# raphaelsulzer/dgnn

Hardware: AMD Instinct MI355X
Metric: tetrahedra/sec (in/out classified), 1M-tet graph at 1/2/4/8 MI355X (higher is better)
Workload: dtype f32 (fp16x2-split products, 22-bit operands; `exact_f32` = bit-faithful fp32 products)

## Files before the change

### dgnn_amd/csrc/fused_ws.hip

```cpp
#include <stdlib.h>

#include "common.h"
#include "fused_common.h"

namespace {
using namespace fused;

typedef float f32x4_t __attribute__((ext_vector_type(4)));
#define H8(v) __builtin_bit_cast(f16x8, v)

constexpr int WS_C = 128;
constexpr int WS_TILE = 32;
constexpr int WS_NP = 8;
template <int CIN> struct WsC {
    static constexpr int NCH = CIN / 16;
    static constexpr int NV = NCH / 4;
    static constexpr int KH = CIN / 32;
    static constexpr int PP = CIN / 8;
    static constexpr int ROWB = 8 * CIN;
    static constexpr int SLOT = WS_TILE * ROWB;
    static constexpr int BP = NCH * 2 * 48 * 16;
};
template <int CIN, int RING> struct WsL {
    static constexpr int OFF_BP = RING * WsC<CIN>::SLOT;
    static constexpr int OFF_ROWF = OFF_BP + WsC<CIN>::BP;
    static constexpr int OFF_CST = OFF_ROWF + RING * WS_TILE * 4;
    static constexpr int OFF_SC = OFF_CST + 3 * WS_C * 4;
    static constexpr int OFF_DC = OFF_SC + 16 + 2 * RING * 4 + 16 + 16;
    static constexpr int OFF_PLOG = OFF_DC + (64 + 64 + 128 + 4) * 4;
    static constexpr int OFF_YS = OFF_PLOG + 2 * 4 * 32 * 8;
    static constexpr int OFF_CMAX = OFF_YS + 2 * 32 * 4;
    static constexpr int OFF_W0S = OFF_CMAX + 4 * 32 * 4;
    static constexpr int OFF_W0 = (OFF_W0S + 32 + 255) & ~255;
    static constexpr int OFF_YT = OFF_W0 + 4 * 4 * 2 * 64 * 16;
    static constexpr int SMEM = OFF_SC + 16 + 2 * RING * 4 + 16 + 16;
    static constexpr int SMEM_DEC = OFF_YT + 2 * 4 * 2 * 2 * 64 * 16;
    static_assert(SMEM_DEC <= 160 * 1024, "the LDS of one CU");
};

struct WsDec {
    const float* W0;
    const float* b0;
    const float* scale1;
    const float* shift1;
    const float* W3;
    const float* b3;
    float* logits;
};


__device__ __forceinline__ void st_nt16(float* p, f32x4_t v) { __builtin_nontemporal_store(v, reinterpret_cast<f32x4_t*>(p)); }
typedef uint32_t u32x2_t __attribute__((ext_vector_type(2)));
__device__ __forceinline__ float ub16_lo(uint32_t u) { return __builtin_fabsf(__builtin_bit_cast(float, u << 15)); }
__device__ __forceinline__ float ub16_hi(uint32_t u) { return __builtin_bit_cast(float, (u >> 16) << 15); }
__device__ __forceinline__ uint32_t ub16_enc(float v) {
    const uint32_t b = __builtin_bit_cast(uint32_t, v) & 0x7FFFFFFFu;
    return (b + 0x3FFFu + ((b >> 15) & 1u)) >> 15;
}
__device__ __forceinline__ uint32_t bits(float f) { return __builtin_bit_cast(uint32_t, f); }

constexpr int WS_KNOBS = 1 | (0 << 4);
template <int CIN, int RING, bool DEC, bool IO16 = false>
__global__ void __launch_bounds__(1024) k_sage_fused_ws(const int32_t* __restrict__ rowptr, const int32_t* __restrict__ src, const int32_t* __restrict__ eid,
                                                        int64_t n_dst, const float* __restrict__ x, const float* __restrict__ xdst, int64_t ldx,
                                                        const float* __restrict__ ea, int64_t lde, const float* __restrict__ We, const float* __restrict__ be,
                                                        const float* __restrict__ Wj, const float* __restrict__ bj, const float* __restrict__ Wi,
                                                        const float* __restrict__ scale, const float* __restrict__ shift, int relu, float* __restrict__ out,
                                                        int64_t ldo, int64_t ntiles, int knobs, WsDec dec) {
    static_assert(CIN == 128 || (CIN == 64 && !DEC), "input widths of the shipped model's 128-wide layers");
    static_assert(!IO16 || !DEC, "the decoder-carrying launch of the bf16-storage chain stays with fused_bf16.hip");
    const uint16_t* const x16 = reinterpret_cast<const uint16_t*>(x);
    const uint16_t* const xdst16 = reinterpret_cast<const uint16_t*>(xdst);
    uint16_t* const out16 = reinterpret_cast<uint16_t*>(out);
    typedef WsC<CIN> G;
    constexpr int NCH = G::NCH, NV = G::NV, KH = G::KH, PP = G::PP;
    extern __shared__ __attribute__((aligned(16))) char ws_smem[];
    const bool nt_store = (knobs & 1) != 0;
    typedef WsL<CIN, RING> L;
    char* const ring = ws_smem;
    char* const bpbuf = ws_smem + L::OFF_BP;
    float* const rowf = reinterpret_cast<float*>(ws_smem + L::OFF_ROWF);
    float* const cst = reinterpret_cast<float*>(ws_smem + L::OFF_CST);
    uint32_t* const scbuf = reinterpret_cast<uint32_t*>(ws_smem + L::OFF_SC);
    volatile uint32_t* const ready = reinterpret_cast<volatile uint32_t*>(ws_smem + L::OFF_SC + 16);
    volatile uint32_t* const done = ready + RING;
    volatile uint32_t* const ycnt = done + RING;
    volatile uint32_t* const yfree = ycnt + 2;
    volatile uint32_t* const lcnt = ycnt + 4;
    volatile uint32_t* const ccnt = ycnt + 6;
    float* const dcst = reinterpret_cast<float*>(ws_smem + L::OFF_DC);
    float* const plog = reinterpret_cast<float*>(ws_smem + L::OFF_PLOG);
    float* const ysc = reinterpret_cast<float*>(ws_smem + L::OFF_YS);
    uint32_t* const cmax = reinterpret_cast<uint32_t*>(ws_smem + L::OFF_CMAX);
    uint32_t* const w0max = reinterpret_cast<uint32_t*>(ws_smem + L::OFF_W0S);
    float* const w0inv = reinterpret_cast<float*>(ws_smem + L::OFF_W0S + 16);
    char* const w0buf = ws_smem + L::OFF_W0;
    char* const ytile = ws_smem + L::OFF_YT;
    typedef __attribute__((address_space(3))) volatile uint32_t lds_vu32;
    auto wait_for = [&](volatile uint32_t* ctr, uint32_t target) {
        asm volatile("" ::: "memory");
        lds_vu32* c3 = (lds_vu32*)ctr;
        while ((int32_t)(__builtin_amdgcn_readfirstlane((int)*c3) - (int)target) < 0) __builtin_amdgcn_s_sleep(1);
        asm volatile("" ::: "memory");
    };
    const int lane = lane_id(), w = wave_id_uniform();
    const int jcol = lane & 15, tq = lane >> 4;

    const int nwg = gridDim.x, xcd = blockIdx.x & 7, slot_ = blockIdx.x >> 3, wg_per_xcd = (nwg + 7 - xcd) >> 3;
    const int64_t per = (ntiles + 7) / 8, t_lo = xcd * per, t_hi = min(ntiles, t_lo + per);
    int64_t my_n = 0;
    if (t_lo + slot_ < t_hi) my_n = (t_hi - t_lo - slot_ + wg_per_xcd - 1) / wg_per_xcd;
    auto tile_of = [&](int64_t it) { return t_lo + slot_ + it * wg_per_xcd; };

    if (threadIdx.x == 0) scbuf[0] = 0u;
    if (threadIdx.x < 2 * RING + 8) ready[threadIdx.x] = 0u;
    if constexpr (DEC) {
        for (int n_ = threadIdx.x; n_ < 64; n_ += blockDim.x) {
            const float s1 = dec.scale1 ? dec.scale1[n_] : 1.f, h1 = dec.scale1 ? dec.shift1[n_] : 0.f;
            dcst[n_] = s1;
            dcst[64 + n_] = __fmaf_rn(dec.b0[n_], s1, h1);
            dcst[128 + n_] = dec.W3[n_];
            dcst[192 + n_] = dec.W3[64 + n_];
        }
        if (threadIdx.x < 2) dcst[256 + threadIdx.x] = dec.b3[threadIdx.x];
        if (threadIdx.x < 4 * WS_TILE) cmax[threadIdx.x] = 0u;
        if (threadIdx.x < 4) w0max[threadIdx.x] = 0u;
    }
    __syncthreads();
    if constexpr (DEC) {
#pragma unroll
        for (int hb = 0; hb < 4; ++hb) {
            uint32_t m0 = 0u;
            for (int e = threadIdx.x; e < 16 * WS_C; e += blockDim.x) m0 = umax(m0, absbits(dec.W0[hb * 16 * WS_C + e]));
            m0 = wave_umax(m0);
            if ((threadIdx.x & 63) == 0) atomicMax(&w0max[hb], m0);
        }
    }
    {
        uint32_t me = 0u;
        for (int e = threadIdx.x; e < CIN * FE; e += blockDim.x) me = umax(me, absbits(We[e]));
        for (int e = threadIdx.x; e < CIN; e += blockDim.x) me = umax(me, absbits(be[e]));
        me = wave_umax(me);
        if (lane == 0) atomicMax(&scbuf[0], me);
    }
    for (int c = threadIdx.x; c < WS_C; c += blockDim.x) {
        cst[c] = bj ? bj[c] : 0.f;
        cst[WS_C + c] = scale ? scale[c] : 1.f;
        cst[2 * WS_C + c] = scale ? shift[c] : 0.f;
    }
    __syncthreads();
    float sWe, inv_sWe;
    pow2_scales(scbuf[0], sWe, inv_sWe);
    constexpr bool LINE_OWN = !IO16 && NV == 2;
    auto chan = [](int j, int cb) { return LINE_OWN ? ((cb >> 2) * 64 + 4 * j + (cb & 3)) : NCH * j + cb; };
    for (int e = threadIdx.x; e < NCH * 48; e += blockDim.x) {
        const int cb = e / 48, gj = e - cb * 48, g = gj >> 4, j = gj & 15;
        const int c = chan(j, cb);
        uint32_t ph[4], pl[4];
#pragma unroll
        for (int d = 0; d < 4; ++d) {
            float v[2];
#pragma unroll
            for (int u = 0; u < 2; ++u) {
                const int k = 8 * g + 2 * d + u;
                v[u] = k < FE ? We[(int64_t)c * FE + k] : (k == FE ? be[c] : 0.f);
            }
            split2h(v[0] * sWe, v[1] * sWe, ph[d], pl[d]);
        }
        uint4* dst = reinterpret_cast<uint4*>(bpbuf + ((cb * 2) * 48 + gj) * 16);
        dst[0] = make_uint4(ph[0], ph[1], ph[2], ph[3]);
        dst[48] = make_uint4(pl[0], pl[1], pl[2], pl[3]);
    }

    auto stage_b = [&](uint32_t t, int hb, int b) {
        wait_for(ycnt + (t & 1), 8u * (t / 2 + 1));
        int ln = lane;
        asm volatile("" : "+v"(ln));
        const char* yt = ytile + ((t & 1) << 14) + ((b * 128 + ln) << 4);
        const char* wp = w0buf + ((hb * 512 + ln) << 4);
        const float inv = ysc[(t & 1) * WS_TILE + 16 * b + (ln & 15)] * w0inv[hb];
        f32x4_t hs = {0.f, 0.f, 0.f, 0.f};
#pragma unroll
        for (int s = 0; s < 4; ++s) {
            const f16x8 w0h = H8(*reinterpret_cast<const uint4*>(wp + (s << 11))), w0l = H8(*reinterpret_cast<const uint4*>(wp + (s << 11) + 1024));
            const f16x8 yh = H8(*reinterpret_cast<const uint4*>(yt + (s << 12))), yl = H8(*reinterpret_cast<const uint4*>(yt + (s << 12) + 1024));
            hs = __builtin_amdgcn_mfma_f32_16x16x32_f16(w0l, yh, hs, 0, 0, 0);
            hs = __builtin_amdgcn_mfma_f32_16x16x32_f16(w0h, yl, hs, 0, 0, 0);
            hs = __builtin_amdgcn_mfma_f32_16x16x32_f16(w0h, yh, hs, 0, 0, 0);
        }
        asm volatile("s_waitcnt lgkmcnt(0)" ::: "memory");
        if (lane == 0) atomicAdd(const_cast<uint32_t*>(yfree + (t & 1)), 1u);
#pragma unroll
        for (int i = 0; i < 4; ++i) hs[i] *= inv;
        const int u0 = 16 * hb + 4 * (ln >> 4);
        float l0 = 0.f, l1 = 0.f;
#pragma unroll
        for (int i = 0; i < 4; ++i) {
            const float hv = fmaxf(__fmaf_rn(hs[i], dcst[u0 + i], dcst[64 + u0 + i]), 0.f);
            l0 = __fmaf_rn(hv, dcst[128 + u0 + i], l0);
            l1 = __fmaf_rn(hv, dcst[192 + u0 + i], l1);
        }
        l0 = cross_row_sum(l0);
        l1 = cross_row_sum(l1);
        if (ln < 16) *reinterpret_cast<float2*>(plog + (((t & 1) * 4 + hb) * WS_TILE + 16 * b + ln) * 2) = make_float2(l0, l1);
        asm volatile("s_waitcnt lgkmcnt(0)" ::: "memory");
        if (lane == 0) atomicAdd(const_cast<uint32_t*>(lcnt + (t & 1)), 1u);
    };

    const int bsel = (knobs >> 4) & 3;
    auto b_on_consumers = [&](uint32_t t) { return bsel == 0 ? false : bsel == 1 ? (t & 1) == 0 : bsel == 2 ? (t & 3) != 3 : true; };

    if (w >= WS_NP) {
        const int cw = w - WS_NP;
        const int col = 16 * cw + jcol;
        uint32_t mw = 0u;
#pragma unroll
        for (int s = 0; s < 2 * KH; ++s) {
            const float* wr = (s < KH ? Wj : Wi) + (int64_t)col * CIN + 32 * (s % KH) + 8 * tq;
            const f32x4_t r0 = *reinterpret_cast<const f32x4_t*>(wr), r1 = *reinterpret_cast<const f32x4_t*>(wr + 4);
#pragma unroll
            for (int i = 0; i < 4; ++i) mw = umax(mw, umax(absbits(r0[i]), absbits(r1[i])));
        }
        float sW, inv_sW;
        pow2_scales(wave_umax(mw), sW, inv_sW);
        f16x8 wh[2 * KH], wl[2 * KH];
#pragma unroll
        for (int s = 0; s < 2 * KH; ++s) {
            const float* wr = (s < KH ? Wj : Wi) + (int64_t)col * CIN + 32 * (s % KH) + 8 * tq;
            const f32x4_t r0 = *reinterpret_cast<const f32x4_t*>(wr), r1 = *reinterpret_cast<const f32x4_t*>(wr + 4);
            uint32_t ph[4], pl[4];
            split2h(r0[0] * sW, r0[1] * sW, ph[0], pl[0]);
            split2h(r0[2] * sW, r0[3] * sW, ph[1], pl[1]);
            split2h(r1[0] * sW, r1[1] * sW, ph[2], pl[2]);
            split2h(r1[2] * sW, r1[3] * sW, ph[3], pl[3]);
            wh[s] = pack8h(ph);
            wl[s] = pack8h(pl);
        }
        if constexpr (DEC) {
#pragma unroll
            for (int u = 0; u < 2; ++u) {
                const int hb = 2 * (cw & 1) + u, ks = cw >> 1;
                float sW0, inv_sW0;
                pow2_scales(w0max[hb], sW0, inv_sW0);
                if (ks == 0 && lane == 0) w0inv[hb] = inv_sW0;
                const float* wr = dec.W0 + (int64_t)(16 * hb + jcol) * WS_C + 32 * ks + 8 * tq;
                const f32x4_t r0 = *reinterpret_cast<const f32x4_t*>(wr), r1 = *reinterpret_cast<const f32x4_t*>(wr + 4);
                uint32_t ph[4], pl[4];
                split2h(r0[0] * sW0, r0[1] * sW0, ph[0], pl[0]);
                split2h(r0[2] * sW0, r0[3] * sW0, ph[1], pl[1]);
                split2h(r1[0] * sW0, r1[1] * sW0, ph[2], pl[2]);
                split2h(r1[2] * sW0, r1[3] * sW0, ph[3], pl[3]);
                uint4* dst = reinterpret_cast<uint4*>(w0buf + (((hb * 4 + ks) * 128 + lane) << 4));
                dst[0] = make_uint4(ph[0], ph[1], ph[2], ph[3]);
                dst[64] = make_uint4(pl[0], pl[1], pl[2], pl[3]);
            }
        }
        __syncthreads();
        const int c0 = 16 * cw + 4 * tq;
        const int64_t n_it = my_n + (DEC ? 3 : 0);
        f32x4_t yp[2] = {{0.f, 0.f, 0.f, 0.f}, {0.f, 0.f, 0.f, 0.f}}, yn[2] = {yp[0], yp[1]};
        for (int64_t it = 1; it <= n_it; ++it) {
            if constexpr (DEC) {
                if (cw == 0 && it >= 4) {
                    const uint32_t t = (uint32_t)(it - 4);
                    wait_for(lcnt + (t & 1), 8u * (t / 2 + 1));
                    if (lane < WS_TILE) {
                        float s0 = dcst[256], s1 = dcst[257];
#pragma unroll
                        for (int q = 0; q < 4; ++q) {
                            const float* pq = plog + (((t & 1) * 4 + q) * WS_TILE + lane) * 2;
                            s0 += pq[0];
                            s1 += pq[1];
                        }
                        const int64_t cell = tile_of(t) * WS_TILE + lane;
                        if (cell < n_dst) *reinterpret_cast<float2*>(dec.logits + cell * 2) = make_float2(s0, s1);
                    }
                }
            }
            if (it >= 1 && it <= my_n) {
                const int sl = (int)((it - 1) % RING);
                wait_for(ready + sl, (uint32_t)(WS_NP * ((it - 1) / RING + 1)));
                const char* tb = ring + sl * G::SLOT;
                f32x4_t acc[2] = {{0.f, 0.f, 0.f, 0.f}, {0.f, 0.f, 0.f, 0.f}};
                int key = jcol;
                asm volatile("" : "+v"(key));
                f16x8 xh[2][2], xl[2][2];
                auto ld_step = [&](int s, int set) {
#pragma unroll
                    for (int b = 0; b < 2; ++b) {
                        const char* rp = tb + (16 * b + jcol) * G::ROWB;
                        xh[set][b] = H8(*reinterpret_cast<const uint4*>(rp + (((4 * s + tq) ^ key) << 4)));
                        xl[set][b] = H8(*reinterpret_cast<const uint4*>(rp + (((2 * PP + 4 * s + tq) ^ key) << 4)));
                    }
                };
                ld_step(0, 0);
#pragma unroll
                for (int s = 0; s < 2 * KH; ++s) {
                    const int set = s & 1;
                    if (s + 1 < 2 * KH) ld_step(s + 1, set ^ 1);
                    __builtin_amdgcn_sched_barrier(0);
#pragma unroll
                    for (int b = 0; b < 2; ++b) acc[b] = __builtin_amdgcn_mfma_f32_16x16x32_f16(wl[s], xh[set][b], acc[b], 0, 0, 0);
#pragma unroll
                    for (int b = 0; b < 2; ++b) acc[b] = __builtin_amdgcn_mfma_f32_16x16x32_f16(wh[s], xl[set][b], acc[b], 0, 0, 0);
#pragma unroll
                    for (int b = 0; b < 2; ++b) acc[b] = __builtin_amdgcn_mfma_f32_16x16x32_f16(wh[s], xh[set][b], acc[b], 0, 0, 0);
                    __builtin_amdgcn_sched_barrier(0);
                }
                float invr[2];
#pragma unroll
                for (int b = 0; b < 2; ++b) invr[b] = rowf[sl * WS_TILE + 16 * b + jcol] * inv_sW;
                asm volatile("s_waitcnt lgkmcnt(0)" ::: "memory");
                if (lane == 0) atomicAdd(const_cast<uint32_t*>(done + sl), 1u);
                const f32x4_t bb = *reinterpret_cast<const f32x4_t*>(cst + c0), sc = *reinterpret_cast<const f32x4_t*>(cst + WS_C + c0),
                              sh = *reinterpret_cast<const f32x4_t*>(cst + 2 * WS_C + c0);
                f32x4_t yv[2];
#pragma unroll
                for (int b = 0; b < 2; ++b) {
#pragma unroll
                    for (int i = 0; i < 4; ++i) {
                        float t_ = __fmaf_rn(acc[b][i], invr[b], bb[i]);
                        t_ = __fmaf_rn(t_, sc[i], sh[i]);
                        yv[b][i] = relu ? fmaxf(t_, 0.f) : t_;
                    }
                }
                if constexpr (!DEC) {
                    const int64_t cell0 = tile_of(it - 1) * WS_TILE;
#pragma unroll
                    for (int b = 0; b < 2; ++b) {
                        const int64_t cell = cell0 + 16 * b + jcol;
                        if (cell < n_dst) {
                            if constexpr (IO16) {
                                const u32x2_t pk = {ub16_enc(yv[b][0]) | (ub16_enc(yv[b][1]) << 16), ub16_enc(yv[b][2]) | (ub16_enc(yv[b][3]) << 16)};
                                if (nt_store) __builtin_nontemporal_store(pk, reinterpret_cast<u32x2_t*>(out16 + cell * ldo + c0));
                                else *reinterpret_cast<u32x2_t*>(out16 + cell * ldo + c0) = pk;
                            } else {
                                if (nt_store) st_nt16(out + cell * ldo + c0, yv[b]);
                                else *reinterpret_cast<f32x4_t*>(out + cell * ldo + c0) = yv[b];
                            }
                        }
                    }
                } else {
                    const uint32_t t = (uint32_t)(it - 1);
                    uint32_t* cm = cmax + (t & 3) * WS_TILE + jcol;
#pragma unroll
                    for (int b = 0; b < 2; ++b) {
                        const float my = fmaxf(fmaxf(fabsf(yv[b][0]), fabsf(yv[b][1])), fmaxf(fabsf(yv[b][2]), fabsf(yv[b][3])));
                        atomicMax(cm + 16 * b, ((t / 4 + 1) << 8) | (bits(my) >> 23));
                    }
                    asm volatile("s_waitcnt lgkmcnt(0)" ::: "memory");
                    if (lane == 0) atomicAdd(const_cast<uint32_t*>(ccnt + (t & 1)), 1u);
                    yn[0] = yv[0], yn[1] = yv[1];
                }
            }
            if constexpr (DEC) {
                if (it >= 2 && it <= my_n + 1) {
                    const uint32_t t = (uint32_t)(it - 2);
                    wait_for(ccnt + (t & 1), 8u * (t / 2 + 1));
                    wait_for(yfree + (t & 1), 8u * (t / 2));
                    int ln = lane;
                    asm volatile("" : "+v"(ln));
                    const uint32_t* cm = cmax + (t & 3) * WS_TILE + (ln & 15);
                    char* yt = ytile + ((t & 1) << 14) + ((cw >> 1) << 12) + (((ln & 15) + 16 * (2 * (cw & 1) + (ln >> 5))) << 4) + (((ln >> 4) & 1) << 3);
#pragma unroll
                    for (int b = 0; b < 2; ++b) {
                        float sY, inv_sY;
                        pow2_scales((cm[16 * b] & 255u) << 23, sY, inv_sY);
                        uint32_t ph[2], pl[2];
                        split2h(yp[b][0] * sY, yp[b][1] * sY, ph[0], pl[0]);
                        split2h(yp[b][2] * sY, yp[b][3] * sY, ph[1], pl[1]);
                        *reinterpret_cast<uint2*>(yt + (b << 11)) = make_uint2(ph[0], ph[1]);
                        *reinterpret_cast<uint2*>(yt + (b << 11) + 1024) = make_uint2(pl[0], pl[1]);
                        if (cw == 0 && ln < 16) ysc[(t & 1) * WS_TILE + 16 * b + ln] = inv_sY;
                    }
                    asm volatile("s_waitcnt lgkmcnt(0)" ::: "memory");
                    if (lane == 0) atomicAdd(const_cast<uint32_t*>(ycnt + (t & 1)), 1u);
                }
                yp[0] = yn[0], yp[1] = yn[1];
                if (it >= 3 && it <= my_n + 2 && b_on_consumers((uint32_t)(it - 3))) stage_b((uint32_t)(it - 3), cw & 3, cw >> 2);
            }
        }
        return;
    }

    __syncthreads();
    const int p = w;
    const int P0 = NCH * jcol;
    const int Q0 = 4 * jcol;
    auto load_rp = [&](int64_t it, int& vb) {
        if (it < my_n) {
            const int64_t i0 = tile_of(it) * WS_TILE + 4 * p;
            const int nv = (int)max((int64_t)0, min((int64_t)4, n_dst - i0));
            vb = nv > 0 ? rowptr[i0 + (lane < nv ? lane : nv)] : 0;
        }
    };
    auto load_idx = [&](int64_t it, int vb, bool& reg, int& vsrc, int& veid) {
        reg = false;
        if (it < my_n) {
            const int64_t i0 = tile_of(it) * WS_TILE + 4 * p;
            const int nv = (int)max((int64_t)0, min((int64_t)4, n_dst - i0));
            if (nv > 0) {
                const int b0 = __builtin_amdgcn_readfirstlane(vb);
                reg = __all(vb == b0 + 4 * (lane < nv ? lane : nv)) != 0;
                if (reg) {
                    const int k_me = b0 + (lane < 4 * nv ? lane : 4 * nv - 1);
                    vsrc = src[k_me];
                    veid = eid ? eid[k_me] : k_me;
                }
            }
        }
    };
    int vb1 = 0, vb2 = 0, vsrc1 = 0, veid1 = 0;
    bool reg1 = false;
    load_rp(0, vb1);
    load_rp(1, vb2);
    load_idx(0, vb1, reg1, vsrc1, veid1);

    for (int64_t it = 0; it < my_n + (DEC ? 3 : 0); ++it) {
        int nv = 0, sl = 0, tl = 0, vsrc = 0, veid = 0;
        bool regular = false;
        f32x4_t xo[NV], q0, q1, rr[4][NV];
        uint32_t xo16[NCH / 2], rr16[4][NCH / 2];
        int64_t cell = 0;
        auto own_row = [&]() {
            if constexpr (IO16) {
                const uint16_t* rp0 = xdst16 + cell * ldx + P0;
                if constexpr (NCH == 8) {
                    const uint4 u = *reinterpret_cast<const uint4*>(rp0);
                    xo16[0] = u.x, xo16[1] = u.y, xo16[2] = u.z, xo16[3] = u.w;
                } else {
                    const uint2 u = *reinterpret_cast<const uint2*>(rp0);
                    xo16[0] = u.x, xo16[1] = u.y;
                }
            } else {
                const float* rp0 = xdst + cell * ldx + (LINE_OWN ? Q0 : P0);
#pragma unroll
                for (int v = 0; v < NV; ++v) xo[v] = *reinterpret_cast<const f32x4_t*>(rp0 + (LINE_OWN ? 64 : 4) * v);
            }
        };
        auto neighbour_rows = [&]() {
            const float* er = ea + (int64_t)__shfl(veid, jcol) * lde;
            q0 = *reinterpret_cast<const f32x4_t*>(er + 8 * (tq < 2 ? tq : 2));
            q1 = *reinterpret_cast<const f32x4_t*>(er + 8 * (tq < 1 ? tq : 1) + 4);
#pragma unroll
            for (int r = 0; r < 4; ++r) {
                if constexpr (IO16) {
                    const uint16_t* rp = x16 + (int64_t)__shfl(vsrc, tl * 4 + r) * ldx + P0;
                    if constexpr (NCH == 8) {
                        const uint4 u = *reinterpret_cast<const uint4*>(rp);
                        rr16[r][0] = u.x, rr16[r][1] = u.y, rr16[r][2] = u.z, rr16[r][3] = u.w;
                    } else {
                        const uint2 u = *reinterpret_cast<const uint2*>(rp);
                        rr16[r][0] = u.x, rr16[r][1] = u.y;
                    }
                } else {
                    const float* rp = x + (int64_t)__shfl(vsrc, tl * 4 + r) * ldx + (LINE_OWN ? Q0 : P0);
#pragma unroll
                    for (int v = 0; v < NV; ++v) rr[r][v] = *reinterpret_cast<const f32x4_t*>(rp + (LINE_OWN ? 64 : 4) * v);
                }
            }
        };
        if (it < my_n) {
            const int64_t i0 = tile_of(it) * WS_TILE + 4 * p;
            sl = (int)(it % RING);
            nv = (int)max((int64_t)0, min((int64_t)4, n_dst - i0));
            regular = reg1;
            vsrc = vsrc1;
            veid = veid1;
            vb1 = vb2;
            load_idx(it + 1, vb1, reg1, vsrc1, veid1);
            load_rp(it + 2, vb2);
            tl = tq < nv ? tq : nv - 1;
            cell = i0 + tl;
        }
        if constexpr (DEC) {
            if (it < my_n && nv > 0) {
                own_row();
                if (regular) neighbour_rows();
            }
            if (it >= 3 && !b_on_consumers((uint32_t)(it - 3))) stage_b((uint32_t)(it - 3), p & 3, p >> 2);
        }
        if (it < my_n) {
            if (nv > 0) {
                if constexpr (!DEC) own_row();
                float aout[NCH], xv[NCH];
#pragma unroll
                for (int v = 0; v < NV; ++v) {
#pragma unroll
                    for (int i = 0; i < 4; ++i) {
                        if constexpr (IO16) xv[4 * v + i] = (i & 1) ? ub16_hi(xo16[2 * v + (i >> 1)]) : ub16_lo(xo16[2 * v + (i >> 1)]);
                        else xv[4 * v + i] = xo[v][i];
                    }
                }
                if (regular) {
                    if constexpr (!DEC) neighbour_rows();
                    float av[8];
#pragma unroll
                    for (int i = 0; i < 4; ++i) {
                        av[i] = tq < 3 ? q0[i] : 0.f;
                        av[4 + i] = tq < 2 ? q1[i] : 0.f;
                    }
                    if (tq == 2) av[4] = 1.0f;
                    float mf = 0.f;
#pragma unroll
                    for (int i = 0; i < 8; i += 2) mf = fmaxf(fmaxf(mf, fabsf(av[i])), fabsf(av[i + 1]));
                    float sA, inv_sA;
                    pow2_scales(cross_row_umax(bits(mf)), sA, inv_sA);
                    uint32_t ph[4], pl[4];
#pragma unroll
                    for (int d = 0; d < 4; ++d) split2h(av[2 * d] * sA, av[2 * d + 1] * sA, ph[d], pl[d]);
                    float inv_e[4];
#pragma unroll
                    for (int r = 0; r < 4; ++r) inv_e[r] = __shfl(inv_sA, 4 * tq + r);
                    const f16x8 ah = pack8h(ph), al = pack8h(pl);
#pragma unroll
                    for (int c4 = 0; c4 < NCH; c4 += 2) {
                        f16x8 bh[2], bl[2];
                        f32x4_t d[2];
#pragma unroll
                        for (int u = 0; u < 2; ++u) {
                            const char* bp = bpbuf + (((c4 + u) * 2) * 48 + (tq < 3 ? tq : 0) * 16 + jcol) * 16;
                            bh[u] = H8(*reinterpret_cast<const uint4*>(bp));
                            bl[u] = H8(*reinterpret_cast<const uint4*>(bp + 768));
                            d[u] = f32x4_t{0.f, 0.f, 0.f, 0.f};
                        }
#pragma unroll
                        for (int u = 0; u < 2; ++u) d[u] = __builtin_amdgcn_mfma_f32_16x16x32_f16(al, bh[u], d[u], 0, 0, 0);
#pragma unroll
                        for (int u = 0; u < 2; ++u) d[u] = __builtin_amdgcn_mfma_f32_16x16x32_f16(ah, bl[u], d[u], 0, 0, 0);
#pragma unroll
                        for (int u = 0; u < 2; ++u) d[u] = __builtin_amdgcn_mfma_f32_16x16x32_f16(ah, bh[u], d[u], 0, 0, 0);
#pragma unroll
                        for (int u = 0; u < 2; ++u) {
                            const int c8 = c4 + u;
#pragma unroll
                            for (int r = 0; r < 4; ++r) d[u][r] *= inv_e[r];
                            auto nb_ = [&](int r) {
                                if constexpr (IO16) return (c8 & 1) ? ub16_hi(rr16[r][c8 >> 1]) : ub16_lo(rr16[r][c8 >> 1]);
                                else return rr[r][c8 >> 2][c8 & 3];
                            };
                            float a = __fmul_rn(nb_(0), d[u][0]);
#pragma unroll
                            for (int r = 1; r < 4; ++r) a = __fmaf_rn(nb_(r), d[u][r], a);
                            aout[c8] = a * (0.25f * inv_sWe);
                        }
                    }
                } else {
#pragma unroll
                    for (int cb = 0; cb < NCH; ++cb) aout[cb] = 0.f;
                    if (tq < nv) {
                        const int b = rowptr[cell], e_end = rowptr[cell + 1];
                        for (int k = b; k < e_end; ++k) {
                            const int s_ = src[k];
                            const float* ar = ea + (int64_t)(eid ? eid[k] : k) * lde;
#pragma unroll 1
                            for (int cb = 0; cb < NCH; ++cb) {
                                const int c = chan(jcol, cb);
                                float pf = be[c];
                                for (int f = 0; f < FE; ++f) pf = __fmaf_rn(We[(int64_t)c * FE + f], ar[f], pf);
                                const float xs_ = IO16 ? __builtin_bit_cast(float, (uint32_t)x16[(int64_t)s_ * ldx + c] << 15) : x[(int64_t)s_ * ldx + c];
                                aout[cb] = __fadd_rn(aout[cb], __fmul_rn(xs_, pf));
                            }
                        }
                        const float cnt = (float)max(e_end - b, 1);
#pragma unroll
                        for (int cb = 0; cb < NCH; ++cb) aout[cb] = __fdiv_rn(aout[cb], cnt);
                    }
                }
                float ma = 0.f;
#pragma unroll
                for (int i = 0; i < NCH; i += 2) {
                    ma = fmaxf(fmaxf(ma, fabsf(aout[i])), fabsf(aout[i + 1]));
                    ma = fmaxf(fmaxf(ma, fabsf(xv[i])), fabsf(xv[i + 1]));
                }
                float s_, inv_;
                pow2_scales(row16_umax(bits(ma)), s_, inv_);
                const int T = 4 * p + tq;
                wait_for(done + sl, (uint32_t)(8 * (it / RING)));
                if (jcol == 0) rowf[sl * WS_TILE + T] = inv_;
                uint32_t ah_[NCH / 2], al_[NCH / 2], xh_[NCH / 2], xl_[NCH / 2];
#pragma unroll
                for (int d = 0; d < NCH / 2; ++d) {
                    split2h(aout[2 * d] * s_, aout[2 * d + 1] * s_, ah_[d], al_[d]);
                    split2h(xv[2 * d] * s_, xv[2 * d + 1] * s_, xh_[d], xl_[d]);
                }
                char* rowp = ring + sl * G::SLOT + T * G::ROWB;
                const int key = T & 15;
                if constexpr (LINE_OWN) {
                    const int half = (jcol & 1) << 3;
#pragma unroll
                    for (int qd = 0; qd < 2; ++qd) {
                        const int pc = 8 * qd + (jcol >> 1);
                        *reinterpret_cast<uint2*>(rowp + ((pc ^ key) << 4) + half) = make_uint2(ah_[2 * qd], ah_[2 * qd + 1]);
                        *reinterpret_cast<uint2*>(rowp + (((PP + pc) ^ key) << 4) + half) = make_uint2(xh_[2 * qd], xh_[2 * qd + 1]);
                        *reinterpret_cast<uint2*>(rowp + (((2 * PP + pc) ^ key) << 4) + half) = make_uint2(al_[2 * qd], al_[2 * qd + 1]);
                        *reinterpret_cast<uint2*>(rowp + (((3 * PP + pc) ^ key) << 4) + half) = make_uint2(xl_[2 * qd], xl_[2 * qd + 1]);
                    }
                } else if constexpr (NCH == 8) {
                    *reinterpret_cast<uint4*>(rowp + ((jcol ^ key) << 4)) = make_uint4(ah_[0], ah_[1], ah_[2], ah_[3]);
                    *reinterpret_cast<uint4*>(rowp + (((PP + jcol) ^ key) << 4)) = make_uint4(xh_[0], xh_[1], xh_[2], xh_[3]);
                    *reinterpret_cast<uint4*>(rowp + (((2 * PP + jcol) ^ key) << 4)) = make_uint4(al_[0], al_[1], al_[2], al_[3]);
                    *reinterpret_cast<uint4*>(rowp + (((3 * PP + jcol) ^ key) << 4)) = make_uint4(xl_[0], xl_[1], xl_[2], xl_[3]);
                } else {
                    const int pc = jcol >> 1, half = (jcol & 1) << 3;
                    *reinterpret_cast<uint2*>(rowp + ((pc ^ key) << 4) + half) = make_uint2(ah_[0], ah_[1]);
                    *reinterpret_cast<uint2*>(rowp + (((PP + pc) ^ key) << 4) + half) = make_uint2(xh_[0], xh_[1]);
                    *reinterpret_cast<uint2*>(rowp + (((2 * PP + pc) ^ key) << 4) + half) = make_uint2(al_[0], al_[1]);
                    *reinterpret_cast<uint2*>(rowp + (((3 * PP + pc) ^ key) << 4) + half) = make_uint2(xl_[0], xl_[1]);
                }
            } else {
                wait_for(done + sl, (uint32_t)(8 * (it / RING)));
            }
            asm volatile("s_waitcnt lgkmcnt(0)" ::: "memory");
            if (lane == 0) atomicAdd(const_cast<uint32_t*>(ready + sl), 1u);
        }
    }
}

}

int dgnn_ws_enabled() {
    static const int v = getenv("DGNN_WS") ? atoi(getenv("DGNN_WS")) : 1;
    return v;
}

extern "C" int dgnn_wave_specialised_enabled(void) { return dgnn_ws_enabled() != 0 ? 1 : 0; }

int dgnn_sage_layer_fused_ws_try(const LayerCall& c, const DecoderTail& t) {
    const bool dec = t.W0 != nullptr;
    if ((c.c_in != WS_C && !(c.c_in == 64 && !dec)) || c.c_out != WS_C || c.lde != FE || c.ldx % 4 != 0 || (!dec && c.ldo % 4 != 0) ||
        ((((uintptr_t)c.x_src | (uintptr_t)c.x_dst | (uintptr_t)c.edge_attr | (uintptr_t)(dec ? nullptr : c.out) | (uintptr_t)c.Wj | (uintptr_t)c.Wi |
           (uintptr_t)t.W0) % 16) != 0) ||
        (dec && ((uintptr_t)t.logits % 8) != 0))
        return DGNN_E_UNSUPPORTED;
    static const int ws64 = getenv("DGNN_WS_64") ? atoi(getenv("DGNN_WS_64")) : 1;
    if (c.c_in == 64 && !ws64) return DGNN_E_UNSUPPORTED;
    const int64_t ntiles = dgnn_cdiv(c.n_dst, WS_TILE);
    int grid = (int)(ntiles < DGNN_NUM_CU ? ntiles : DGNN_NUM_CU);
    if (grid < 1) grid = 1;
    const WsDec d{t.W0, t.b0, t.scale1, t.shift1, t.W3, t.b3, t.logits};
#define DGNN_WS_GO(C_, D_)                                                                                                                                  \
    do {                                                                                                                                                    \
        static bool attr_[DGNN_MAX_DEVICES] = {};                                                                                                           \
        const size_t sm_ = D_ ? WsL<C_, 2>::SMEM_DEC : WsL<C_, 2>::SMEM;                                                                                    \
        dgnn_allow_dynamic_lds(reinterpret_cast<const void*>(&k_sage_fused_ws<C_, 2, D_>), sm_, attr_);                                                     \
        hipLaunchKernelGGL((k_sage_fused_ws<C_, 2, D_>), dim3(grid), dim3(1024), sm_, c.stream, c.rowptr, c.src, c.eid, c.n_dst, c.x_src, c.x_dst, c.ldx,    \
                           c.edge_attr, c.lde, c.We, c.be, c.Wj, c.bj, c.Wi, c.scale, c.shift, c.relu, c.out, c.ldo, ntiles, WS_KNOBS, d);                  \
    } while (0)
    if (c.c_in == 64) DGNN_WS_GO(64, false);
    else if (dec) DGNN_WS_GO(128, true);
    else DGNN_WS_GO(128, false);
#undef DGNN_WS_GO
    return dgnn_check_launch(dec ? "sage_layer_fused_decoder_fwd(wave-specialised)" : "sage_layer_fused_fwd(wave-specialised)");
}

int dgnn_sage_layer_fused_ws16_try(const LayerCall16& c) {
    static const int on = getenv("DGNN_WS_16") ? atoi(getenv("DGNN_WS_16")) : 1;
    const int nch = c.c_in / 16;
    if (!on || !dgnn_ws_enabled() || (c.c_in != 128 && c.c_in != 64) || c.c_out != WS_C || !c.relu || c.lde != FE || c.ldx % nch != 0 || c.ldo % 4 != 0 ||
        ((((uintptr_t)c.x_src | (uintptr_t)c.x_dst) % (2 * nch)) != 0) || ((uintptr_t)c.out % 8) != 0 ||
        ((((uintptr_t)c.edge_attr | (uintptr_t)c.Wj | (uintptr_t)c.Wi) % 16) != 0))
        return DGNN_E_UNSUPPORTED;
    const int64_t ntiles = dgnn_cdiv(c.n_dst, WS_TILE);
    int grid = (int)(ntiles < DGNN_NUM_CU ? ntiles : DGNN_NUM_CU);
    if (grid < 1) grid = 1;
    const WsDec d{};
    const float* xs = static_cast<const float*>(c.x_src);
    const float* xd = static_cast<const float*>(c.x_dst);
    float* o = reinterpret_cast<float*>(c.out);
    if (c.c_in == 64) {
        static bool attr_[DGNN_MAX_DEVICES] = {};
        const size_t sm_ = WsL<64, 4>::SMEM;
        dgnn_allow_dynamic_lds(reinterpret_cast<const void*>(&k_sage_fused_ws<64, 4, false, true>), sm_, attr_);
        hipLaunchKernelGGL((k_sage_fused_ws<64, 4, false, true>), dim3(grid), dim3(1024), sm_, c.stream, c.rowptr, c.src, c.eid, c.n_dst, xs, xd, c.ldx, c.edge_attr,
                           c.lde, c.We, c.be, c.Wj, c.bj, c.Wi, c.scale, c.shift, c.relu, o, c.ldo, ntiles, WS_KNOBS, d);
    } else {
        static bool attr_[DGNN_MAX_DEVICES] = {};
        const size_t sm_ = WsL<128, 2>::SMEM;
        dgnn_allow_dynamic_lds(reinterpret_cast<const void*>(&k_sage_fused_ws<128, 2, false, true>), sm_, attr_);
        hipLaunchKernelGGL((k_sage_fused_ws<128, 2, false, true>), dim3(grid), dim3(1024), sm_, c.stream, c.rowptr, c.src, c.eid, c.n_dst, xs, xd, c.ldx, c.edge_attr,
                           c.lde, c.We, c.be, c.Wj, c.bj, c.Wi, c.scale, c.shift, c.relu, o, c.ldo, ntiles, WS_KNOBS, d);
    }
    return dgnn_check_launch("sage_layer_fused_fwd_bf16(wave-specialised)");
}
```

Baseline: 735.5 million.

## Double tile size to 64 rows for the bf16 64-wide wave-specialised layer

For the 64->128 bf16-storage layer, the tile grows from 32 to 64 destination rows and the ring shrinks from 4 to 2 slots. Each producer wave now gathers two 4-row groups per iteration, and consumer waves issue twice as many MFMA blocks per tile. This amortises the per-tile handshakes and weight fragment reuse over more rows. The cost is fewer tiles to spread across CUs, less pipelining depth in the ring, and a larger producer code path with more register pressure.

```diff
diff --git a/dgnn_amd/csrc/fused_ws.hip b/dgnn_amd/csrc/fused_ws.hip
--- a/dgnn_amd/csrc/fused_ws.hip
+++ b/dgnn_amd/csrc/fused_ws.hip
@@ -10,21 +10,24 @@
 #define H8(v) __builtin_bit_cast(f16x8, v)
 
 constexpr int WS_C = 128;
-constexpr int WS_TILE = 32;
 constexpr int WS_NP = 8;
-template <int CIN> struct WsC {
+template <int CIN, bool IO16 = false> struct WsC {
+    static constexpr int TILE = (CIN == 64 && IO16) ? 64 : 32;
+    static constexpr int NG = TILE / 32;
+    static constexpr int NB = TILE / 16;
     static constexpr int NCH = CIN / 16;
     static constexpr int NV = NCH / 4;
     static constexpr int KH = CIN / 32;
     static constexpr int PP = CIN / 8;
     static constexpr int ROWB = 8 * CIN;
-    static constexpr int SLOT = WS_TILE * ROWB;
+    static constexpr int SLOT = TILE * ROWB;
     static constexpr int BP = NCH * 2 * 48 * 16;
 };
-template <int CIN, int RING> struct WsL {
-    static constexpr int OFF_BP = RING * WsC<CIN>::SLOT;
-    static constexpr int OFF_ROWF = OFF_BP + WsC<CIN>::BP;
-    static constexpr int OFF_CST = OFF_ROWF + RING * WS_TILE * 4;
+template <int CIN, int RING, bool IO16 = false> struct WsL {
+    typedef WsC<CIN, IO16> G;
+    static constexpr int OFF_BP = RING * G::SLOT;
+    static constexpr int OFF_ROWF = OFF_BP + G::BP;
+    static constexpr int OFF_CST = OFF_ROWF + RING * G::TILE * 4;
     static constexpr int OFF_SC = OFF_CST + 3 * WS_C * 4;
     static constexpr int OFF_DC = OFF_SC + 16 + 2 * RING * 4 + 16 + 16;
     static constexpr int OFF_PLOG = OFF_DC + (64 + 64 + 128 + 4) * 4;
@@ -72,11 +75,11 @@
     const uint16_t* const x16 = reinterpret_cast<const uint16_t*>(x);
     const uint16_t* const xdst16 = reinterpret_cast<const uint16_t*>(xdst);
     uint16_t* const out16 = reinterpret_cast<uint16_t*>(out);
-    typedef WsC<CIN> G;
-    constexpr int NCH = G::NCH, NV = G::NV, KH = G::KH, PP = G::PP;
+    typedef WsC<CIN, IO16> G;
+    constexpr int NCH = G::NCH, NV = G::NV, KH = G::KH, PP = G::PP, NG = G::NG, NB = G::NB;
     extern __shared__ __attribute__((aligned(16))) char ws_smem[];
     const bool nt_store = (knobs & 1) != 0;
-    typedef WsL<CIN, RING> L;
+    typedef WsL<CIN, RING, IO16> L;
     char* const ring = ws_smem;
     char* const bpbuf = ws_smem + L::OFF_BP;
     float* const rowf = reinterpret_cast<float*>(ws_smem + L::OFF_ROWF);
@@ -123,7 +126,7 @@
             dcst[192 + n_] = dec.W3[64 + n_];
         }
         if (threadIdx.x < 2) dcst[256 + threadIdx.x] = dec.b3[threadIdx.x];
-        if (threadIdx.x < 4 * WS_TILE) cmax[threadIdx.x] = 0u;
+        if (threadIdx.x < 4 * G::TILE) cmax[threadIdx.x] = 0u;
         if (threadIdx.x < 4) w0max[threadIdx.x] = 0u;
     }
     __syncthreads();
@@ -178,7 +181,7 @@
         asm volatile("" : "+v"(ln));
         const char* yt = ytile + ((t & 1) << 14) + ((b * 128 + ln) << 4);
         const char* wp = w0buf + ((hb * 512 + ln) << 4);
-        const float inv = ysc[(t & 1) * WS_TILE + 16 * b + (ln & 15)] * w0inv[hb];
+        const float inv = ysc[(t & 1) * G::TILE + 16 * b + (ln & 15)] * w0inv[hb];
         f32x4_t hs = {0.f, 0.f, 0.f, 0.f};
 #pragma unroll
         for (int s = 0; s < 4; ++s) {
@@ -202,7 +205,7 @@
         }
         l0 = cross_row_sum(l0);
         l1 = cross_row_sum(l1);
-        if (ln < 16) *reinterpret_cast<float2*>(plog + (((t & 1) * 4 + hb) * WS_TILE + 16 * b + ln) * 2) = make_float2(l0, l1);
+        if (ln < 16) *reinterpret_cast<float2*>(plog + (((t & 1) * 4 + hb) * G::TILE + 16 * b + ln) * 2) = make_float2(l0, l1);
         asm volatile("s_waitcnt lgkmcnt(0)" ::: "memory");
         if (lane == 0) atomicAdd(const_cast<uint32_t*>(lcnt + (t & 1)), 1u);
     };
@@ -264,15 +267,15 @@
                 if (cw == 0 && it >= 4) {
                     const uint32_t t = (uint32_t)(it - 4);
                     wait_for(lcnt + (t & 1), 8u * (t / 2 + 1));
-                    if (lane < WS_TILE) {
+                    if (lane < G::TILE) {
                         float s0 = dcst[256], s1 = dcst[257];
 #pragma unroll
                         for (int q = 0; q < 4; ++q) {
-                            const float* pq = plog + (((t & 1) * 4 + q) * WS_TILE + lane) * 2;
+                            const float* pq = plog + (((t & 1) * 4 + q) * G::TILE + lane) * 2;
                             s0 += pq[0];
                             s1 += pq[1];
                         }
-                        const int64_t cell = tile_of(t) * WS_TILE + lane;
+                        const int64_t cell = tile_of(t) * G::TILE + lane;
                         if (cell < n_dst) *reinterpret_cast<float2*>(dec.logits + cell * 2) = make_float2(s0, s1);
                     }
                 }
@@ -281,42 +284,46 @@
                 const int sl = (int)((it - 1) % RING);
                 wait_for(ready + sl, (uint32_t)(WS_NP * ((it - 1) / RING + 1)));
                 const char* tb = ring + sl * G::SLOT;
-                f32x4_t acc[2] = {{0.f, 0.f, 0.f, 0.f}, {0.f, 0.f, 0.f, 0.f}};
+                f32x4_t acc[NB];
+#pragma unroll
+                for (int b = 0; b < NB; ++b) acc[b] = f32x4_t{0.f, 0.f, 0.f, 0.f};
                 int key = jcol;
                 asm volatile("" : "+v"(key));
+                constexpr int UPS = NB / 2, NU = 2 * KH * UPS;
                 f16x8 xh[2][2], xl[2][2];
-                auto ld_step = [&](int s, int set) {
+                auto ld_unit = [&](int u, int set) {
+                    const int s = u / UPS, b0 = 2 * (u % UPS);
 #pragma unroll
                     for (int b = 0; b < 2; ++b) {
-                        const char* rp = tb + (16 * b + jcol) * G::ROWB;
+                        const char* rp = tb + (16 * (b0 + b) + jcol) * G::ROWB;
                         xh[set][b] = H8(*reinterpret_cast<const uint4*>(rp + (((4 * s + tq) ^ key) << 4)));
                         xl[set][b] = H8(*reinterpret_cast<const uint4*>(rp + (((2 * PP + 4 * s + tq) ^ key) << 4)));
                     }
                 };
-                ld_step(0, 0);
-#pragma unroll
-                for (int s = 0; s < 2 * KH; ++s) {
-                    const int set = s & 1;
-                    if (s + 1 < 2 * KH) ld_step(s + 1, set ^ 1);
+                ld_unit(0, 0);
+#pragma unroll
+                for (int u = 0; u < NU; ++u) {
+                    const int set = u & 1, s = u / UPS, b0 = 2 * (u % UPS);
+                    if (u + 1 < NU) ld_unit(u + 1, set ^ 1);
                     __builtin_amdgcn_sched_barrier(0);
 #pragma unroll
-                    for (int b = 0; b < 2; ++b) acc[b] = __builtin_amdgcn_mfma_f32_16x16x32_f16(wl[s], xh[set][b], acc[b], 0, 0, 0);
-#pragma unroll
-                    for (int b = 0; b < 2; ++b) acc[b] = __builtin_amdgcn_mfma_f32_16x16x32_f16(wh[s], xl[set][b], acc[b], 0, 0, 0);
-#pragma unroll
-                    for (int b = 0; b < 2; ++b) acc[b] = __builtin_amdgcn_mfma_f32_16x16x32_f16(wh[s], xh[set][b], acc[b], 0, 0, 0);
+                    for (int b = 0; b < 2; ++b) acc[b0 + b] = __builtin_amdgcn_mfma_f32_16x16x32_f16(wl[s], xh[set][b], acc[b0 + b], 0, 0, 0);
+#pragma unroll
+                    for (int b = 0; b < 2; ++b) acc[b0 + b] = __builtin_amdgcn_mfma_f32_16x16x32_f16(wh[s], xl[set][b], acc[b0 + b], 0, 0, 0);
+#pragma unroll
+                    for (int b = 0; b < 2; ++b) acc[b0 + b] = __builtin_amdgcn_mfma_f32_16x16x32_f16(wh[s], xh[set][b], acc[b0 + b], 0, 0, 0);
                     __builtin_amdgcn_sched_barrier(0);
                 }
-                float invr[2];
-#pragma unroll
-                for (int b = 0; b < 2; ++b) invr[b] = rowf[sl * WS_TILE + 16 * b + jcol] * inv_sW;
+                float invr[NB];
+#pragma unroll
+                for (int b = 0; b < NB; ++b) invr[b] = rowf[sl * G::TILE + 16 * b + jcol] * inv_sW;
                 asm volatile("s_waitcnt lgkmcnt(0)" ::: "memory");
                 if (lane == 0) atomicAdd(const_cast<uint32_t*>(done + sl), 1u);
                 const f32x4_t bb = *reinterpret_cast<const f32x4_t*>(cst + c0), sc = *reinterpret_cast<const f32x4_t*>(cst + WS_C + c0),
                               sh = *reinterpret_cast<const f32x4_t*>(cst + 2 * WS_C + c0);
-                f32x4_t yv[2];
-#pragma unroll
-                for (int b = 0; b < 2; ++b) {
+                f32x4_t yv[NB];
+#pragma unroll
+                for (int b = 0; b < NB; ++b) {
 #pragma unroll
                     for (int i = 0; i < 4; ++i) {
                         float t_ = __fmaf_rn(acc[b][i], invr[b], bb[i]);
@@ -325,9 +332,9 @@
                     }
                 }
                 if constexpr (!DEC) {
-                    const int64_t cell0 = tile_of(it - 1) * WS_TILE;
-#pragma unroll
-                    for (int b = 0; b < 2; ++b) {
+                    const int64_t cell0 = tile_of(it - 1) * G::TILE;
+#pragma unroll
+                    for (int b = 0; b < NB; ++b) {
                         const int64_t cell = cell0 + 16 * b + jcol;
                         if (cell < n_dst) {
                             if constexpr (IO16) {
@@ -342,7 +349,7 @@
                     }
                 } else {
                     const uint32_t t = (uint32_t)(it - 1);
-                    uint32_t* cm = cmax + (t & 3) * WS_TILE + jcol;
+                    uint32_t* cm = cmax + (t & 3) * G::TILE + jcol;
 #pragma unroll
                     for (int b = 0; b < 2; ++b) {
                         const float my = fmaxf(fmaxf(fabsf(yv[b][0]), fabsf(yv[b][1])), fmaxf(fabsf(yv[b][2]), fabsf(yv[b][3])));
@@ -360,7 +367,7 @@
                     wait_for(yfree + (t & 1), 8u * (t / 2));
                     int ln = lane;
                     asm volatile("" : "+v"(ln));
-                    const uint32_t* cm = cmax + (t & 3) * WS_TILE + (ln & 15);
+                    const uint32_t* cm = cmax + (t & 3) * G::TILE + (ln & 15);
                     char* yt = ytile + ((t & 1) << 14) + ((cw >> 1) << 12) + (((ln & 15) + 16 * (2 * (cw & 1) + (ln >> 5))) << 4) + (((ln >> 4) & 1) << 3);
 #pragma unroll
                     for (int b = 0; b < 2; ++b) {
@@ -371,7 +378,7 @@
                         split2h(yp[b][2] * sY, yp[b][3] * sY, ph[1], pl[1]);
                         *reinterpret_cast<uint2*>(yt + (b << 11)) = make_uint2(ph[0], ph[1]);
                         *reinterpret_cast<uint2*>(yt + (b << 11) + 1024) = make_uint2(pl[0], pl[1]);
-                        if (cw == 0 && ln < 16) ysc[(t & 1) * WS_TILE + 16 * b + ln] = inv_sY;
+                        if (cw == 0 && ln < 16) ysc[(t & 1) * G::TILE + 16 * b + ln] = inv_sY;
                     }
                     asm volatile("s_waitcnt lgkmcnt(0)" ::: "memory");
                     if (lane == 0) atomicAdd(const_cast<uint32_t*>(ycnt + (t & 1)), 1u);
@@ -387,9 +394,219 @@
     const int p = w;
     const int P0 = NCH * jcol;
     const int Q0 = 4 * jcol;
+    if constexpr (NG > 1) {
+        static_assert(NG == 2 && NCH == 4 && IO16 && !DEC, "the 64 -> 128 layer of the bf16-storage chain");
+        auto load_rp = [&](int64_t it, int& vb) {
+            if (it < my_n) {
+                const int64_t i0 = tile_of(it) * G::TILE + 8 * p;
+                const int nv = (int)max((int64_t)0, min((int64_t)8, n_dst - i0));
+                vb = nv > 0 ? rowptr[i0 + (lane < nv ? lane : nv)] : 0;
+            }
+        };
+        auto load_idx = [&](int64_t it, int vb, bool (&reg)[NG], int& vsrc, int& veid) {
+            reg[0] = reg[1] = false;
+            if (it < my_n) {
+                const int64_t i0 = tile_of(it) * G::TILE + 8 * p;
+                int b_me = 0, n_me = 0;
+#pragma unroll
+                for (int g = 0; g < NG; ++g) {
+                    const int nv = (int)max((int64_t)0, min((int64_t)4, n_dst - i0 - 4 * g));
+                    if (nv > 0) {
+                        const int bg = __builtin_amdgcn_readlane(vb, 4 * g), l = lane - 4 * g;
+                        reg[g] = __all(l < 0 || l > nv || vb == bg + 4 * l) != 0;
+                        if (reg[g] && ((lane >> 4) & 1) == g) b_me = bg, n_me = 4 * nv;
+                    }
+                }
+                if (n_me > 0) {
+                    const int k_me = b_me + ((lane & 15) < n_me ? (lane & 15) : n_me - 1);
+                    vsrc = src[k_me];
+                    veid = eid ? eid[k_me] : k_me;
+                }
+            }
+        };
+        int vb1 = 0, vb2 = 0, vsrc1 = 0, veid1 = 0;
+        bool reg1[NG] = {};
+        load_rp(0, vb1);
+        load_rp(1, vb2);
+        load_idx(0, vb1, reg1, vsrc1, veid1);
+
+        for (int64_t it = 0; it < my_n; ++it) {
+            const int64_t i0 = tile_of(it) * G::TILE + 8 * p;
+            const int sl = (int)(it % RING), vsrc = vsrc1, veid = veid1;
+            int nv[NG], tl[NG];
+            bool regular[NG];
+            int64_t cell[NG];
+#pragma unroll
+            for (int g = 0; g < NG; ++g) {
+                nv[g] = (int)max((int64_t)0, min((int64_t)4, n_dst - i0 - 4 * g));
+                regular[g] = reg1[g];
+                tl[g] = tq < nv[g] ? tq : nv[g] - 1;
+                cell[g] = i0 + 4 * g + tl[g];
+            }
+            vb1 = vb2;
+            load_idx(it + 1, vb1, reg1, vsrc1, veid1);
+            load_rp(it + 2, vb2);
+            f32x4_t q0[NG], q1[NG];
+            uint2 xo16[NG], rr16[NG][4];
+            auto own_row = [&](int g) { xo16[g] = *reinterpret_cast<const uint2*>(xdst16 + cell[g] * ldx + P0); };
+            auto neighbour_rows = [&](int g) {
+                const float* er = ea + (int64_t)__shfl(veid, 16 * g + jcol) * lde;
+                q0[g] = *reinterpret_cast<const f32x4_t*>(er + 8 * (tq < 2 ? tq : 2));
+                q1[g] = *reinterpret_cast<const f32x4_t*>(er + 8 * (tq < 1 ? tq : 1) + 4);
+#pragma unroll
+                for (int r = 0; r < 4; ++r) rr16[g][r] = *reinterpret_cast<const uint2*>(x16 + (int64_t)__shfl(vsrc, 16 * g + tl[g] * 4 + r) * ldx + P0);
+            };
+            auto own_values = [&](int g, float (&xv)[NCH]) {
+#pragma unroll
+                for (int i = 0; i < 4; ++i) {
+                    const uint32_t u = (i >> 1) ? xo16[g].y : xo16[g].x;
+                    xv[i] = (i & 1) ? ub16_hi(u) : ub16_lo(u);
+                }
+            };
+            auto mean_regular = [&](int g, float (&aout)[NCH]) {
+                float av[8];
+#pragma unroll
+                for (int i = 0; i < 4; ++i) {
+                    av[i] = tq < 3 ? q0[g][i] : 0.f;
+                    av[4 + i] = tq < 2 ? q1[g][i] : 0.f;
+                }
+                if (tq == 2) av[4] = 1.0f;
+                float mf = 0.f;
+#pragma unroll
+                for (int i = 0; i < 8; i += 2) mf = fmaxf(fmaxf(mf, fabsf(av[i])), fabsf(av[i + 1]));
+                float sA, inv_sA;
+                pow2_scales(cross_row_umax(bits(mf)), sA, inv_sA);
+                uint32_t ph[4], pl[4];
+#pragma unroll
+                for (int d = 0; d < 4; ++d) split2h(av[2 * d] * sA, av[2 * d + 1] * sA, ph[d], pl[d]);
+                float inv_e[4];
+#pragma unroll
+                for (int r = 0; r < 4; ++r) inv_e[r] = __shfl(inv_sA, 4 * tq + r);
+                const f16x8 ah = pack8h(ph), al = pack8h(pl);
+#pragma unroll
+                for (int c4 = 0; c4 < NCH; c4 += 2) {
+                    f16x8 bh[2], bl[2];
+                    f32x4_t d[2];
+#pragma unroll
+                    for (int u = 0; u < 2; ++u) {
+                        const char* bp = bpbuf + (((c4 + u) * 2) * 48 + (tq < 3 ? tq : 0) * 16 + jcol) * 16;
+                        bh[u] = H8(*reinterpret_cast<const uint4*>(bp));
+                        bl[u] = H8(*reinterpret_cast<const uint4*>(bp + 768));
+                        d[u] = f32x4_t{0.f, 0.f, 0.f, 0.f};
+                    }
+#pragma unroll
+                    for (int u = 0; u < 2; ++u) d[u] = __builtin_amdgcn_mfma_f32_16x16x32_f16(al, bh[u], d[u], 0, 0, 0);
+#pragma unroll
+                    for (int u = 0; u < 2; ++u) d[u] = __builtin_amdgcn_mfma_f32_16x16x32_f16(ah, bl[u], d[u], 0, 0, 0);
+#pragma unroll
+                    for (int u = 0; u < 2; ++u) d[u] = __builtin_amdgcn_mfma_f32_16x16x32_f16(ah, bh[u], d[u], 0, 0, 0);
+#pragma unroll
+                    for (int u = 0; u < 2; ++u) {
+                        const int c8 = c4 + u;
+#pragma unroll
+                        for (int r = 0; r < 4; ++r) d[u][r] *= inv_e[r];
+                        auto nb_ = [&](int r) {
+                            const uint32_t v = (c8 >> 1) ? rr16[g][r].y : rr16[g][r].x;
+                            return (c8 & 1) ? ub16_hi(v) : ub16_lo(v);
+                        };
+                        float a = __fmul_rn(nb_(0), d[u][0]);
+#pragma unroll
+                        for (int r = 1; r < 4; ++r) a = __fmaf_rn(nb_(r), d[u][r], a);
+                        aout[c8] = a * (0.25f * inv_sWe);
+                    }
+                }
+            };
+            auto mean_generic = [&](int g, float (&aout)[NCH]) {
+#pragma unroll
+                for (int cb = 0; cb < NCH; ++cb) aout[cb] = 0.f;
+                if (tq < nv[g]) {
+                    const int b = rowptr[cell[g]], e_end = rowptr[cell[g] + 1];
+                    for (int k = b; k < e_end; ++k) {
+                        const int s_ = src[k];
+                        const float* ar = ea + (int64_t)(eid ? eid[k] : k) * lde;
+#pragma unroll 1
+                        for (int cb = 0; cb < NCH; ++cb) {
+                            const int c = chan(jcol, cb);
+                            float pf = be[c];
+                            for (int f = 0; f < FE; ++f) pf = __fmaf_rn(We[(int64_t)c * FE + f], ar[f], pf);
+                            const float xs_ = __builtin_bit_cast(float, (uint32_t)x16[(int64_t)s_ * ldx + c] << 15);
+                            aout[cb] = __fadd_rn(aout[cb], __fmul_rn(xs_, pf));
+                        }
+                    }
+                    const float cnt = (float)max(e_end - b, 1);
+#pragma unroll
+                    for (int cb = 0; cb < NCH; ++cb) aout[cb] = __fdiv_rn(aout[cb], cnt);
+                }
+            };
+            auto row_scale = [&](const float (&aout)[NCH], const float (&xv)[NCH], float& s_, float& inv_) {
+                float ma = 0.f;
+#pragma unroll
+                for (int i = 0; i < NCH; i += 2) {
+                    ma = fmaxf(fmaxf(ma, fabsf(aout[i])), fabsf(aout[i + 1]));
+                    ma = fmaxf(fmaxf(ma, fabsf(xv[i])), fabsf(xv[i + 1]));
+                }
+                pow2_scales(row16_umax(bits(ma)), s_, inv_);
+            };
+            auto park = [&](int g, const float (&aout)[NCH], const float (&xv)[NCH], float s_, float inv_) {
+                const int T = 8 * p + 4 * g + tq;
+                if (jcol == 0) rowf[sl * G::TILE + T] = inv_;
+                uint32_t ah_[2], al_[2], xh_[2], xl_[2];
+#pragma unroll
+                for (int d = 0; d < 2; ++d) {
+                    split2h(aout[2 * d] * s_, aout[2 * d + 1] * s_, ah_[d], al_[d]);
+                    split2h(xv[2 * d] * s_, xv[2 * d + 1] * s_, xh_[d], xl_[d]);
+                }
+                char* rowp = ring + sl * G::SLOT + T * G::ROWB;
+                const int key = T & 15, pc = jcol >> 1, half = (jcol & 1) << 3;
+                *reinterpret_cast<uint2*>(rowp + ((pc ^ key) << 4) + half) = make_uint2(ah_[0], ah_[1]);
+                *reinterpret_cast<uint2*>(rowp + (((PP + pc) ^ key) << 4) + half) = make_uint2(xh_[0], xh_[1]);
+                *reinterpret_cast<uint2*>(rowp + (((2 * PP + pc) ^ key) << 4) + half) = make_uint2(al_[0], al_[1]);
+                *reinterpret_cast<uint2*>(rowp + (((3 * PP + pc) ^ key) << 4) + half) = make_uint2(xl_[0], xl_[1]);
+            };
+            if (regular[0] && regular[1]) {
+                own_row(0);
+                own_row(1);
+                neighbour_rows(0);
+                neighbour_rows(1);
+                __builtin_amdgcn_sched_barrier(0);
+                float aout[NG][NCH], xv[NG][NCH], s_[NG], inv_[NG];
+#pragma unroll
+                for (int g = 0; g < NG; ++g) {
+                    own_values(g, xv[g]);
+                    mean_regular(g, aout[g]);
+                    row_scale(aout[g], xv[g], s_[g], inv_[g]);
+                }
+                wait_for(done + sl, (uint32_t)(8 * (it / RING)));
+#pragma unroll
+                for (int g = 0; g < NG; ++g) park(g, aout[g], xv[g], s_[g], inv_[g]);
+            } else {
+                wait_for(done + sl, (uint32_t)(8 * (it / RING)));
+#pragma unroll
+                for (int g = 0; g < NG; ++g) {
+                    if (nv[g] > 0) {
+                        float aout[NCH], xv[NCH], s_, inv_;
+                        own_row(g);
+                        own_values(g, xv);
+                        if (regular[g]) {
+                            neighbour_rows(g);
+                            mean_regular(g, aout);
+                        } else {
+                            mean_generic(g, aout);
+                        }
+                        row_scale(aout, xv, s_, inv_);
+                        park(g, aout, xv, s_, inv_);
+                    }
+                }
+            }
+            asm volatile("s_waitcnt lgkmcnt(0)" ::: "memory");
+            if (lane == 0) atomicAdd(const_cast<uint32_t*>(ready + sl), 1u);
+        }
+        return;
+    }
+
     auto load_rp = [&](int64_t it, int& vb) {
         if (it < my_n) {
-            const int64_t i0 = tile_of(it) * WS_TILE + 4 * p;
+            const int64_t i0 = tile_of(it) * G::TILE + 4 * p;
             const int nv = (int)max((int64_t)0, min((int64_t)4, n_dst - i0));
             vb = nv > 0 ? rowptr[i0 + (lane < nv ? lane : nv)] : 0;
         }
@@ -397,7 +614,7 @@
     auto load_idx = [&](int64_t it, int vb, bool& reg, int& vsrc, int& veid) {
         reg = false;
         if (it < my_n) {
-            const int64_t i0 = tile_of(it) * WS_TILE + 4 * p;
+            const int64_t i0 = tile_of(it) * G::TILE + 4 * p;
             const int nv = (int)max((int64_t)0, min((int64_t)4, n_dst - i0));
             if (nv > 0) {
                 const int b0 = __builtin_amdgcn_readfirstlane(vb);
@@ -461,7 +678,7 @@
             }
         };
         if (it < my_n) {
-            const int64_t i0 = tile_of(it) * WS_TILE + 4 * p;
+            const int64_t i0 = tile_of(it) * G::TILE + 4 * p;
             sl = (int)(it % RING);
             nv = (int)max((int64_t)0, min((int64_t)4, n_dst - i0));
             regular = reg1;
@@ -577,7 +794,7 @@
                 pow2_scales(row16_umax(bits(ma)), s_, inv_);
                 const int T = 4 * p + tq;
                 wait_for(done + sl, (uint32_t)(8 * (it / RING)));
-                if (jcol == 0) rowf[sl * WS_TILE + T] = inv_;
+                if (jcol == 0) rowf[sl * G::TILE + T] = inv_;
                 uint32_t ah_[NCH / 2], al_[NCH / 2], xh_[NCH / 2], xl_[NCH / 2];
 #pragma unroll
                 for (int d = 0; d < NCH / 2; ++d) {
@@ -635,7 +852,7 @@
         return DGNN_E_UNSUPPORTED;
     static const int ws64 = getenv("DGNN_WS_64") ? atoi(getenv("DGNN_WS_64")) : 1;
     if (c.c_in == 64 && !ws64) return DGNN_E_UNSUPPORTED;
-    const int64_t ntiles = dgnn_cdiv(c.n_dst, WS_TILE);
+    const int64_t ntiles = dgnn_cdiv(c.n_dst, WsC<128>::TILE);
     int grid = (int)(ntiles < DGNN_NUM_CU ? ntiles : DGNN_NUM_CU);
     if (grid < 1) grid = 1;
     const WsDec d{t.W0, t.b0, t.scale1, t.shift1, t.W3, t.b3, t.logits};
@@ -661,7 +878,7 @@
         ((((uintptr_t)c.x_src | (uintptr_t)c.x_dst) % (2 * nch)) != 0) || ((uintptr_t)c.out % 8) != 0 ||
         ((((uintptr_t)c.edge_attr | (uintptr_t)c.Wj | (uintptr_t)c.Wi) % 16) != 0))
         return DGNN_E_UNSUPPORTED;
-    const int64_t ntiles = dgnn_cdiv(c.n_dst, WS_TILE);
+    const int64_t ntiles = dgnn_cdiv(c.n_dst, c.c_in == 64 ? WsC<64, true>::TILE : WsC<128, true>::TILE);
     int grid = (int)(ntiles < DGNN_NUM_CU ? ntiles : DGNN_NUM_CU);
     if (grid < 1) grid = 1;
     const WsDec d{};
@@ -670,13 +887,13 @@
     float* o = reinterpret_cast<float*>(c.out);
     if (c.c_in == 64) {
         static bool attr_[DGNN_MAX_DEVICES] = {};
-        const size_t sm_ = WsL<64, 4>::SMEM;
-        dgnn_allow_dynamic_lds(reinterpret_cast<const void*>(&k_sage_fused_ws<64, 4, false, true>), sm_, attr_);
-        hipLaunchKernelGGL((k_sage_fused_ws<64, 4, false, true>), dim3(grid), dim3(1024), sm_, c.stream, c.rowptr, c.src, c.eid, c.n_dst, xs, xd, c.ldx, c.edge_attr,
+        const size_t sm_ = WsL<64, 2, true>::SMEM;
+        dgnn_allow_dynamic_lds(reinterpret_cast<const void*>(&k_sage_fused_ws<64, 2, false, true>), sm_, attr_);
+        hipLaunchKernelGGL((k_sage_fused_ws<64, 2, false, true>), dim3(grid), dim3(1024), sm_, c.stream, c.rowptr, c.src, c.eid, c.n_dst, xs, xd, c.ldx, c.edge_attr,
                            c.lde, c.We, c.be, c.Wj, c.bj, c.Wi, c.scale, c.shift, c.relu, o, c.ldo, ntiles, WS_KNOBS, d);
     } else {
         static bool attr_[DGNN_MAX_DEVICES] = {};
-        const size_t sm_ = WsL<128, 2>::SMEM;
+        const size_t sm_ = WsL<128, 2, true>::SMEM;
         dgnn_allow_dynamic_lds(reinterpret_cast<const void*>(&k_sage_fused_ws<128, 2, false, true>), sm_, attr_);
         hipLaunchKernelGGL((k_sage_fused_ws<128, 2, false, true>), dim3(grid), dim3(1024), sm_, c.stream, c.rowptr, c.src, c.eid, c.n_dst, xs, xd, c.ldx, c.edge_attr,
                            c.lde, c.We, c.be, c.Wj, c.bj, c.Wi, c.scale, c.shift, c.relu, o, c.ldo, ntiles, WS_KNOBS, d);
```

Measured after the change: 732.5 million. About the same (-0.4%).
